# anuunchin/learned-quantization

Measured on AMD Instinct MI355X. Metric: images/sec training with fake-quant layer, CIFAR-10 bs=256, 1/2/4/8 MI355X, higher is better.
Workload: dtype f32; 1 GPU; fake-quant fwd+bwd (split) on conv-activation batch 256x3x224x224 fp32 per GPU, per_channel scales, lambda=1e-11; per_gpu_batch=256, global_batch=256, parallelism=dp1, buffer_sets=4, launch=eager

## Files before the change

learned_quantization_amd/csrc/lq_common.hpp:

```cpp
#ifndef LQ_COMMON_HPP_
#define LQ_COMMON_HPP_
#include <hip/hip_runtime.h>
#include <stdint.h>

#include "lq_hip.h"
#include "lq_fastdiv.hpp"

namespace lq {

constexpr int kBlock = 256;
constexpr int kWavesPerBlock = kBlock / 64;
constexpr float kEpsF32 = 1.1920928955078125e-07f;
constexpr int64_t kPeriodic4Min = 4ll << 20;
constexpr int64_t kNtBytes = 64ll << 20;

struct Params {
    const float* P;
    const float* s;
    const float* dy;
    float* out;
    void* q;
    int q_dtype;
    float lam;
    int tmode;
    const float* mb;
    const uint32_t* ties;
    const float* c_dev;
    float c_scale;
    int accum;
    uint32_t* pa;
    uint32_t* pb;
    double* pc;
    int64_t outer, G, inner;
    int direct;
    float* e0;
    float* e1;
    double ecount;
    float* out_perm;
    const float* dy_perm;
    float* dp_out;
    uint32_t perm_hw, perm_ci, perm_co;
};

__device__ __forceinline__ uint32_t perm_index(const Params& p, int64_t i) {
    const uint32_t iu = (uint32_t)i;
    const uint32_t t = iu / p.perm_co, o = iu - t * p.perm_co;
    const uint32_t h = t / p.perm_ci, c = t - h * p.perm_ci;
    return (o * p.perm_ci + c) * p.perm_hw + h;
}

struct FlatIdx {
    FastDiv inner, G;
};

struct Ctx {
    float s;
    float r;
    int fast;
    float k0;
    float k1;
    float lam_hi;
    int sure_ok;
};

template <typename TB, typename TC>
struct AccT {
    uint32_t a;
    TB b;
    TC c;
};
using Acc = AccT<uint32_t, double>;
using AccW = AccT<double, double>;

enum OpKind {
    OP_FWD = 0,
    OP_BWD = 1,
    OP_FUSED = 2,
    OP_MAXBIN_FWD = 3,
    OP_MAXBIN_BWD = 4,
    OP_DIFF_FWD = 5,
    OP_DIFF_BWD = 6,
    OP_QONLY = 7,
    OP_FWD_PERM = 8,
    OP_BWD_PERM = 9,
    OP_DIFF_BWD_V = 10,
};

}

#endif
```

learned_quantization_amd/csrc/lq_kernels.hip:

```cpp
#include <hip/hip_runtime.h>
#include <hip/hip_ext.h>
#include <stdarg.h>
#include <stdlib.h>
#include <stdint.h>
#include <stdio.h>
#include <string.h>

#include <new>
#include <algorithm>
#include <vector>

#include "lq_hip.h"

#include "lq_batch.hpp"
#include "lq_stream2.hpp"
#include "lq_pack.hpp"

namespace lq {

enum Mode { MODE_ROW_BIG = 0, MODE_ROW_SMALL = 1, MODE_COL = 2 };

constexpr int64_t kColRbFused = 48;
constexpr int64_t kColRbBwd = 128;

struct Plan {
    int mode;
    int64_t R, L;
    int bs;
    int CH;
    int64_t nc;
    int lpr_log2;
    int64_t C, rps, ysplit;
    int per4;
    int64_t np;
    int64_t np_ws;
    int64_t gstride, n1, stride1, n2;
};

static int64_t ceil_div(int64_t a, int64_t b) { return (a + b - 1) / b; }

#ifdef LQ_DEV_KNOBS
static int knob_env(const char* name, int dflt) {
    const char* e = getenv(name);
    return e ? atoi(e) : dflt;
}
#define LQ_KNOB(var, name, dflt) static const int var = knob_env(name, dflt)
#else
#define LQ_KNOB(var, name, dflt) constexpr int var = (dflt)
#endif

static bool flat_cols_ok(int64_t C) { return C == 8 || C == 16 || C == 32 || C == 64; }
static int64_t colx_max_inner() {
    LQ_KNOB(v, "LQ_TUNE_COLX_INNER", 200);
    return v;
}
static int64_t periodic_target() {
    LQ_KNOB(v, "LQ_TUNE_PER_NB", 2048);
    return v > 0 ? v : 2048;
}
static int64_t periodic_blocks(int64_t C) { return C * ((periodic_target() + C / 2) / C); }

static int64_t row_chunks(int64_t L, int64_t CH) {
    int64_t nc = ceil_div(L, CH);
    const int64_t r = L % CH;
    if (nc > 1 && r != 0 && r * 8 <= CH) nc -= 1;
    return nc;
}

static Plan make_plan(int64_t outer, int64_t G, int64_t inner, int force_bs = 0) {
    Plan pl;
    memset(&pl, 0, sizeof(pl));
    const int64_t N = outer * G * inner;
    int64_t R, L, f_outer;
    bool col = false;
    if (G == 1) {
        R = 1;
        L = N;
        f_outer = 1;
    } else {
        R = outer * G;
        L = inner;
        f_outer = outer;
        LQ_KNOB(colx, "LQ_TUNE_COLX", 1);
        const bool short_rows_many_layers = colx && inner >= 16 && inner < colx_max_inner() && outer >= 32 && (G * inner) % 32 == 0 &&
                                            G * inner > 64 && (double)N >= (double)kPeriodic4Min && !(inner % 4 == 0 && (inner & (inner - 1)) == 0);
        if ((inner < 16 && outer > 1) || short_rows_many_layers) {
            const int64_t C = G * inner;
            int64_t RB;
            int64_t nby = 0;
            int per4 = 0;
            if (C <= 64 && (double)outer * (double)C >= (double)kPeriodic4Min) {
                per4 = 1;
                nby = periodic_blocks(C);
                const int64_t k = 64 / C;
                RB = ceil_div(ceil_div(outer, nby), 4 * k) * 4 * k;
            } else if (C <= 64) {
                const int64_t k = 64 / C;
                RB = ceil_div(ceil_div(16384, C), 4 * k) * 4 * k;
                const int64_t rb_par = ceil_div(ceil_div(outer, 1024), 4 * k) * 4 * k;
                if (rb_par < RB) RB = rb_par;
            } else {
                RB = ceil_div(outer * ceil_div(C, 256), 512);
                RB = ceil_div(RB, 16) * 16;
                if (RB > 128) RB = 128;
                if ((double)outer * (double)C >= (double)kPeriodic4Min) RB = kColRbFused;
                if (short_rows_many_layers && ceil_div(outer, kColRbFused) * C > 2 * R) RB = kColRbBwd;
            }
            if (RB > outer) RB = outer;
            if (!nby) nby = ceil_div(outer, RB);
            if (nby * C <= R || (short_rows_many_layers && nby * C <= 2 * R)) {
                col = true;
                pl.mode = MODE_COL;
                pl.C = C;
                pl.rps = RB;
                pl.ysplit = nby;
                pl.per4 = per4;
                pl.np = nby * C;
                if (per4 && flat_cols_ok(C)) {
                    const int64_t fb = ceil_div(ceil_div(outer * C, 4) + 1, (int64_t)kFlatColsBlock * 2);
                    if (fb * C > pl.np) pl.np = fb * C;
                }
                if (C > 64 && C <= 256 && (double)outer * (double)C >= (double)kPeriodic4Min && periodic_blocks(C) * C > pl.np)
                    pl.np = periodic_blocks(C) * C;
                pl.gstride = inner;
                pl.n1 = nby;
                pl.stride1 = C;
                pl.n2 = inner;
            }
        }
    }
    if (!col) {
        pl.R = R;
// ... 53 lines not shown
static int check_hip(const char* what) {
    hipError_t e = hipGetLastError();
    if (e != hipSuccess) return fail(LQ_EHIP, "%s: %s", what, hipGetErrorString(e));
    return LQ_OK;
}

static bool aligned(const void* p, size_t a) { return (reinterpret_cast<uintptr_t>(p) % a) == 0; }

static int check_desc(int64_t outer, int64_t G, int64_t inner) {
    if (outer <= 0 || G <= 0 || inner <= 0) return fail(LQ_EINVAL, "descriptor extents must be positive (outer=%lld G=%lld inner=%lld)", (long long)outer, (long long)G, (long long)inner);
    const double n = (double)outer * (double)G * (double)inner;
    if (n > 9.0e15) return fail(LQ_EINVAL, "tensor too large");
    return LQ_OK;
}

static size_t ws_bytes_for(const Plan& pl) {
    size_t np = (size_t)(pl.np_ws > pl.np ? pl.np_ws : pl.np);
    np = (np + 63) / 64 * 64;
    return np * 16 + 256;
}

static int bind_ws(Params& p, const Plan& pl, void* ws, size_t ws_bytes) {
    if (!ws) return fail(LQ_EWORKSPACE, "workspace is NULL (need %zu bytes)", ws_bytes_for(pl));
    if (!aligned(ws, 16)) return fail(LQ_EALIGN, "workspace must be 16-byte aligned");
    if (ws_bytes < ws_bytes_for(pl)) return fail(LQ_EWORKSPACE, "workspace too small: %zu < %zu bytes", ws_bytes, ws_bytes_for(pl));
    size_t np = ((size_t)(pl.np_ws > pl.np ? pl.np_ws : pl.np) + 63) / 64 * 64;
    p.pa = reinterpret_cast<uint32_t*>(ws);
    p.pb = p.pa + np;
    p.pc = reinterpret_cast<double*>(p.pb + np);
    return LQ_OK;
}

static int row_small_lpr_log2_vec(int64_t L) {
    const int64_t l4 = L / 4;
    int lg = 0;
    while ((1 << lg) < l4 && lg < 6) ++lg;
    return lg;
}
static bool row_small_vec(const Plan& pl, const void* P, const void* dy, const void* out) {
    return pl.L % 4 == 0 && pl.L >= 8 && aligned(P, 16) && (!dy || aligned(dy, 16)) && (!out || aligned(out, 16));
}

static void col_variant(const Plan& pl, const void* P, const void* dy, const void* out, int& variant, int64_t& nbx,
                        bool allow_periodic4 = true) {
    const bool al16 = aligned(P, 16) && (!dy || aligned(dy, 16)) && (!out || aligned(out, 16));
    const double bytes = (double)pl.C * (double)pl.ysplit * (double)pl.rps * 4.0;
    if (pl.C <= 64) {
        variant = (allow_periodic4 && pl.per4 && al16) ? (bytes >= (double)kNtBytes ? 7 : 6) : 0;
        nbx = 1;
    } else if (pl.C % 4 == 0 && aligned(P, 16) && (!dy || aligned(dy, 16)) && (!out || aligned(out, 16))) {
        variant = ((double)pl.C * (double)pl.ysplit * (double)pl.rps * 4.0 >= (double)kNtBytes) ? 5 : 4;
        nbx = ceil_div(pl.C, 256);
    } else {
        variant = 1;
        nbx = ceil_div(pl.C, 64);
    }
}


#ifdef LQ_DEV_KNOBS
constexpr bool kDevKnobs = true;
#else
constexpr bool kDevKnobs = false;
#endif

template <int OP>
static int launch_stream2_impl(Plan& pl, const Params& p, hipStream_t st);

template <int OP>
static int launch_stream2(Plan& pl, const Params& p, hipStream_t st) {
    if constexpr (OP == OP_FWD || OP == OP_BWD || OP == OP_FUSED) return launch_stream2_impl<OP>(pl, p, st);
    else return 0;
}

template <int OP>
static int launch_stream2_impl(Plan& pl, const Params& p, hipStream_t st) {
    using O = OpT<OP>;
    const double numel = (double)p.outer * (double)p.G * (double)p.inner;
    if (numel < (double)kPeriodic4Min) return 0;
    if (p.out_perm || p.dy_perm) return 0;
    FlatIdx fx;
    fx.inner = make_fastdiv((uint32_t)(p.inner < 4294967296ll ? p.inner : 1));
    fx.G = make_fastdiv((uint32_t)(p.G < 4294967296ll ? p.G : 1));
    (void)fx;
    if (pl.mode == MODE_ROW_BIG) {
        if constexpr (OP == OP_FWD) {
            LQ_KNOB(off_rb, "LQ_TUNE_S2", 0);
            const int64_t nn = p.outer * p.G * p.inner;
            const bool poor_fill = (double)pl.L / (double)(pl.nc * pl.CH) < 0.95;
            if (!(off_rb & 256) && (pl.L % 32 != 0 || poor_fill || !(off_rb & 32768)) && aligned(p.P, 16) && aligned(p.out, 16)) {
                const int64_t nv = nn >> 2;
                const int rem = (int)(nn & 3);
                const int64_t blocks = ceil_div(nv + (rem ? 1 : 0), 512);
                if (blocks <= 2147483647ll) {
                    const bool ntb = numel * 4.0 >= (double)kNtBytes;
                    const bool wide = nn >= 4294967296ll;
#define LQ_FLATR(NT_, GM_) hipExtLaunchKernelGGL((k_flat_fwd<OP, 512, NT_, GM_>), dim3((unsigned)blocks), dim3(512), 0, st, g_prof_start, g_prof_stop, 0, p, fx, nv, rem)
                    if (pl.L % 4 == 0) {
                        if (ntb) { if (wide) LQ_FLATR(1, 2); else LQ_FLATR(1, 0); }
                        else LQ_FLATR(0, 0);
                    } else if (!(off_rb & 512) && (double)pl.L / (double)(pl.nc * pl.CH) >= 0.8) {
                        return 0;
                    } else {
                        if (ntb) { if (wide) LQ_FLATR(1, 7); else LQ_FLATR(1, 6); }
                        else LQ_FLATR(0, 6);
                    }
#undef LQ_FLATR
                    return check_hip("flat forward launch") ? -1 : 1;
                }
            }
        } else {
            LQ_KNOB(off_rb, "LQ_TUNE_S2", 0);
            const int nwin = (int)(pl.L % 4 ? (pl.L + 6) / 4 : pl.L / 4);
            const bool al = aligned(p.P, 16) && aligned(p.dy, 16) && (!O::kStore || aligned(p.out, 16));
            LQ_KNOB(win_max, "LQ_TUNE_WIN_MAX", 384);
            const bool wide_ok = pl.L % 4 != 0 && (double)pl.L / 2048.0 < 0.95;
            if (!(off_rb & 128) && pl.bs == 256 && pl.nc == 2 && (nwin <= win_max || wide_ok) && nwin <= 512 && al && !p.direct && pl.R < 4294967296ll) {
                const int64_t blocks = ceil_div(pl.R, (int64_t)kWavesPerBlock);
                if (blocks <= 2147483647ll) {
                    const int64_t n = p.outer * p.G * p.inner;
                    const bool ntb = numel * 4.0 >= (double)kNtBytes;
                    const FastDiv fG = make_fastdiv((uint32_t)p.G);
                    const int64_t f_outer = pl.R / p.G;
                    pl.nc = 1;
                    pl.np = pl.R;
                    pl.gstride = f_outer;
                    pl.n1 = f_outer;
                    pl.stride1 = 1;
                    pl.n2 = 1;
#define LQ_WINB(NT_, V_) hipLaunchKernelGGL((k_row_win<OP, NT_, 6, V_, 1>), dim3((unsigned)blocks), dim3(kBlock), 0, st, p, fG, pl.R, (int)pl.L, n)
                    if (nwin <= 320) { if (ntb) LQ_WINB(1, 5); else LQ_WINB(0, 5); }
                    else if (nwin <= 384) { if (ntb) LQ_WINB(1, 6); else LQ_WINB(0, 6); }
                    else if (nwin <= 448) { if (ntb) LQ_WINB(1, 7); else LQ_WINB(0, 7); }
                    else { if (ntb) LQ_WINB(1, 8); else LQ_WINB(0, 8); }
#undef LQ_WINB
                    return check_hip("row-window launch") ? -1 : 1;
                }
            }
        }
        return 0;
    }
    const bool al16 = aligned(p.P, 16) && (!O::kDy || aligned(p.dy, 16)) && (!O::kStore || aligned(p.out, 16));
    if (!al16) return 0;
    LQ_KNOB(off, "LQ_TUNE_S2", 0);
    const bool nt = numel * 4.0 >= (double)kNtBytes;
    const int64_t n = p.outer * p.G * p.inner;
    if constexpr (OP == OP_FWD) {
        const bool one_group = p.inner % 4 == 0;
        const bool scale4 = p.inner == 1 && p.G % 4 == 0 && aligned(p.s, 16) && !(off & 32);
        const bool scale4u = p.inner == 1 && p.G % 4 != 0 && p.G > 64 && !(off & 8192);
        const bool cols_pow2 = pl.mode == MODE_COL && pl.per4 && flat_cols_ok(pl.C) && !(off & 64);
        const bool straddle = pl.mode == MODE_ROW_SMALL && pl.L >= 4 && pl.L % 4 != 0 && !(off & 256);
        if (straddle) {
            const int64_t nv = n >> 2;
            const int rem = (int)(n & 3);
            const int64_t blocks = ceil_div(nv + (rem ? 1 : 0), 512);
            if (blocks <= 2147483647ll) {
                const bool wide = n >= 4294967296ll;
#define LQ_FLATS(NT_, GM_) hipLaunchKernelGGL((k_flat_fwd<OP, 512, NT_, GM_>), dim3((unsigned)blocks), dim3(512), 0, st, p, fx, nv, rem)
                if (nt) { if (wide) LQ_FLATS(1, 7); else LQ_FLATS(1, 6); }
                else LQ_FLATS(0, 6);
#undef LQ_FLATS
                return check_hip("flat forward launch") ? -1 : 1;
            }
        }
        if (scale4u && !(off & 1)) {
            const int64_t nv = n >> 2;
            const int rem = (int)(n & 3);
            const int64_t blocks = ceil_div(nv + (rem ? 1 : 0), 512);
            if (blocks <= 2147483647ll) {
                const bool wide = n >= 4294967296ll;
#define LQ_FLATU(NT_, GM_) hipLaunchKernelGGL((k_flat_fwd<OP, 512, NT_, GM_>), dim3((unsigned)blocks), dim3(512), 0, st, p, fx, nv, rem)
                if (nt) { if (wide) LQ_FLATU(1, 9); else LQ_FLATU(1, 8); }
                else LQ_FLATU(0, 8);
#undef LQ_FLATU
                return check_hip("flat forward launch") ? -1 : 1;
            }
        }
        LQ_KNOB(gather_on, "LQ_TUNE_GATHER", 1);
        if (gather_on && !(off & 1) && pl.mode == MODE_COL && !one_group && !scale4 && !scale4u && !cols_pow2 && n < 4294967296ll) {
            const int64_t nv = n >> 2;
// ... 252 lines not shown
#undef LQ_WIN
                return check_hip("row-window launch") ? -1 : 1;
            }
        }
        if ((off & 8) || pl.L > 64 || pl.L < 8 || pl.L % 4 != 0) return 0;
        const int lg = row_small_lpr_log2_vec(pl.L);
        LQ_KNOB(tiny_u, "LQ_TUNE_TINY_U", 2);
        int U = (1 << lg) < tiny_u ? (1 << lg) : tiny_u;
        if (U != 2 && U != 4) U = 2;
        const int64_t rows_per_block = (int64_t)kWavesPerBlock * (64 >> lg) * U;
        const int64_t blocks = ceil_div(pl.R, rows_per_block);
        if (blocks > 2147483647ll) return 0;
        if (pl.R >= 4294967296ll) return 0;
        const int gm = (p.outer == 1) ? 0 : 1;
#define LQ_TINY3(NT_, U_, LG_) do { \
            if (gm == 0) hipLaunchKernelGGL((k_row_tiny<OP, NT_, U_, LG_, 0>), dim3((unsigned)blocks), dim3(kBlock), 0, st, p, pl.R, (int)pl.L); \
            else hipLaunchKernelGGL((k_row_tiny<OP, NT_, U_, LG_, 1>), dim3((unsigned)blocks), dim3(kBlock), 0, st, p, pl.R, (int)pl.L); } while (0)
#ifdef LQ_DEV_KNOBS
#define LQ_TINY2(NT_) do { \
            if (lg == 1) LQ_TINY3(NT_, 2, 1); \
            else if (lg == 2) { if (U == 2) LQ_TINY3(NT_, 2, 2); else LQ_TINY3(NT_, 4, 2); } \
            else if (lg == 3) { if (U == 2) LQ_TINY3(NT_, 2, 3); else LQ_TINY3(NT_, 4, 3); } \
            else { if (U == 2) LQ_TINY3(NT_, 2, 4); else LQ_TINY3(NT_, 4, 4); } } while (0)
#else
#define LQ_TINY2(NT_) do { \
            if (lg == 1) LQ_TINY3(NT_, 2, 1); \
            else if (lg == 2) LQ_TINY3(NT_, 2, 2); \
            else if (lg == 3) LQ_TINY3(NT_, 2, 3); \
            else LQ_TINY3(NT_, 2, 4); } while (0)
#endif
        if (nt) LQ_TINY2(1); else LQ_TINY2(0);
#undef LQ_TINY2
#undef LQ_TINY3
        return check_hip("tiny-row launch") ? -1 : 1;
    }
}

template <int OP>
constexpr bool kStreamOp = OP == OP_FWD || OP == OP_BWD || OP == OP_FUSED;

template <int OP>
static int launch_traverse(Plan& pl, const Params& p, hipStream_t st) {
    using O = OpT<OP>;
    if (!kStreamOp<OP> && pl.mode == MODE_ROW_BIG && pl.bs != kBlock) return fail(LQ_EINVAL, "internal: operation %d planned with %d-thread units", OP, pl.bs);
    {
        const int r2 = launch_stream2<OP>(pl, p, st);
        if (r2 < 0) return LQ_EHIP;
        if (r2 > 0) return LQ_OK;
    }
    if (pl.mode == MODE_ROW_BIG) {
        const bool vec = aligned(p.P, 16) && (!O::kDy || aligned(p.dy, 16)) && (!O::kStore || aligned(p.out, 16));
        LQ_KNOB(tune_chunk, "LQ_TUNE_CHUNK", 1);
        LQ_KNOB(forced_bs, "LQ_TUNE_BS", 0);
        if (pl.bs == 512 && vec && tune_chunk && !p.direct && !forced_bs && pl.np_ws >= pl.R * row_chunks(pl.L, 1024)) {
            auto fill = [&](int64_t CH) { return (double)pl.L / (double)(row_chunks(pl.L, CH) * CH); };
            const bool k2_form = (OP == OP_BWD || (OP == OP_FUSED && p.tmode >= 1)) && (double)pl.R * (double)pl.L * 4.0 >= (double)kNtBytes;
            const bool small = k2_form ? (row_chunks(pl.L, 4096) > 1 && fill(1024) > fill(4096) + 0.1) : (fill(1024) > fill(2048) + 0.05);
            if (small) {
                pl.bs = 256;
                pl.CH = 1024;
                pl.nc = row_chunks(pl.L, 1024);
                pl.np = pl.R * pl.nc;
                pl.gstride = pl.nc;
                pl.stride1 = p.G * pl.nc;
                pl.n2 = pl.nc;
            }
        }
        const int64_t units = pl.R * pl.nc;
        if (units > 2147483647ll) return fail(LQ_EINVAL, "too many work units (%lld)", (long long)units);
        const int64_t outer_f = pl.R / p.G;
        const int grid3d = (p.G <= 65535 && outer_f <= 65535 && pl.R == outer_f * p.G) ? 1 : 0;
        const dim3 grid = grid3d ? dim3((unsigned)pl.nc, (unsigned)p.G, (unsigned)outer_f) : dim3((unsigned)units);
        const bool nt = kStreamOp<OP> && vec && (double)pl.R * (double)pl.L * 4.0 >= (double)kNtBytes;
        LQ_KNOB(tune_u2, "LQ_TUNE_U2", -1);
        const bool want_u2 = tune_u2 >= 0 ? tune_u2 == 1 : (OP == OP_BWD || p.tmode >= 1);
        const bool u2 = (OP == OP_BWD || OP == OP_FUSED) && want_u2 && vec && nt && pl.bs == 512;
        auto needs_tail = [&](int64_t CH) {
            const int64_t r = pl.L % CH;
            return pl.L % 4 != 0 || (pl.L > CH && r != 0 && r * 8 <= CH);
        };
        if constexpr (OP == OP_BWD || OP == OP_FUSED) if (u2) {
            const int64_t nc2 = row_chunks(pl.L, (int64_t)pl.bs * 8);
            const dim3 grid2 = grid3d ? dim3((unsigned)nc2, (unsigned)p.G, (unsigned)outer_f) : dim3((unsigned)(pl.R * nc2));
            if (needs_tail((int64_t)pl.bs * 8))
                hipExtLaunchKernelGGL((k_row_stream<OP, 4, 512, 1, 2, 1>), grid2, dim3(512), 0, st, g_prof_start, g_prof_stop, 0, p, pl.L, nc2, grid3d);
            else
                hipExtLaunchKernelGGL((k_row_stream<OP, 4, 512, 1, 2, 0>), grid2, dim3(512), 0, st, g_prof_start, g_prof_stop, 0, p, pl.L, nc2, grid3d);
            pl.CH = pl.bs * 8;
            pl.nc = nc2;
            pl.np = pl.R * nc2;
            pl.gstride = nc2;
            pl.stride1 = p.G * nc2;
            pl.n2 = nc2;
            return check_hip("traversal launch");
        }
        const bool tail1 = needs_tail((int64_t)pl.CH);
#define LQ_LAUNCH_STREAM(VEC_, BS_, NT_) do { \
        constexpr bool kTail0 = kDevKnobs || (VEC_ == 4 && !(OP == OP_FWD && (BS_ != kBlock || NT_ != 0)) && !(OP == OP_BWD && BS_ == 512 && NT_ == 1)); \
        constexpr bool kTail1 = kDevKnobs || !(OP == OP_BWD && VEC_ == 4 && BS_ == 512 && NT_ == 1); \
        if (VEC_ == 1 || tail1) { if constexpr (kTail1) hipExtLaunchKernelGGL((k_row_stream<OP, VEC_, BS_, NT_, 1, 1>), grid, dim3(BS_), 0, st, g_prof_start, g_prof_stop, 0, p, pl.L, pl.nc, grid3d); } \
        else { if constexpr (kTail0) hipExtLaunchKernelGGL((k_row_stream<OP, VEC_, BS_, NT_, 1, 0>), grid, dim3(BS_), 0, st, g_prof_start, g_prof_stop, 0, p, pl.L, pl.nc, grid3d); } } while (0)
        if constexpr (!kStreamOp<OP>) {
            if (vec) LQ_LAUNCH_STREAM(4, 256, 0);
            else LQ_LAUNCH_STREAM(1, 256, 0);
        } else if (!kDevKnobs && OP == OP_FWD && vec && !tail1 && (pl.bs != kBlock || nt)) {
            return fail(LQ_EINVAL, "internal: streaming-size forward of aligned rows reached the row stream");
        } else if (!kDevKnobs && OP == OP_BWD && vec && nt && pl.bs == 512) {
            return fail(LQ_EINVAL, "internal: streaming-size scale gradient reached the one-float4 row stream");
        } else if (vec) {
#ifdef LQ_DEV_KNOBS
            if (pl.bs == 1024) {
                if (nt) LQ_LAUNCH_STREAM(4, 1024, 1);
                else LQ_LAUNCH_STREAM(4, 1024, 0);
            } else
#endif
            if (pl.bs == 512) {
                if (nt) LQ_LAUNCH_STREAM(4, 512, 1);
                else LQ_LAUNCH_STREAM(4, 512, 0);
            } else {
                if (nt) LQ_LAUNCH_STREAM(4, 256, 1);
                else LQ_LAUNCH_STREAM(4, 256, 0);
            }
        } else {
#ifdef LQ_DEV_KNOBS
            if (pl.bs == 1024) LQ_LAUNCH_STREAM(1, 1024, 0);
            else
#endif
            if (pl.bs == 512) LQ_LAUNCH_STREAM(1, 512, 0);
            else LQ_LAUNCH_STREAM(1, 256, 0);
        }
#undef LQ_LAUNCH_STREAM
    } else if (pl.mode == MODE_ROW_SMALL) {
        const bool vec = row_small_vec(pl, p.P, O::kDy ? p.dy : nullptr, O::kStore ? p.out : nullptr);
        const int lg = vec ? row_small_lpr_log2_vec(pl.L) : pl.lpr_log2;
        const int64_t blocks = ceil_div(pl.R, kBlock >> lg);
        if (blocks > 2147483647ll) return fail(LQ_EINVAL, "too many blocks (%lld)", (long long)blocks);
        if (vec) hipLaunchKernelGGL((k_row_small<OP, 4>), dim3((unsigned)blocks), dim3(kBlock), 0, st, p, pl.R, (int)pl.L, lg);
        else hipLaunchKernelGGL((k_row_small<OP, 1>), dim3((unsigned)blocks), dim3(kBlock), 0, st, p, pl.R, (int)pl.L, lg);
    } else {
        int variant;
        int64_t nbx;
        col_variant(pl, p.P, O::kDy ? p.dy : nullptr, O::kStore ? p.out : nullptr, variant, nbx);
        const int64_t blocks = nbx * pl.ysplit;
        if (blocks > 2147483647ll) return fail(LQ_EINVAL, "too many blocks (%lld)", (long long)blocks);
        hipLaunchKernelGGL((k_col<OP>), dim3((unsigned)blocks), dim3(kBlock), 0, st, p, pl.C, pl.rps, nbx, variant, pl.ysplit);
    }
    return check_hip("traversal launch");
}

static bool finalize_cols_single(const FinGeom& f) {
    return finalize_cols_ok(f.groups, f.gstride, f.n1, f.stride1, f.n2) && f.n1 <= 64 && f.n1 * f.groups * f.n2 >= 131072;
}

template <int OP, bool COLS = true>
static int launch_finalize(const Params& p, FinGeom f, hipStream_t st) {
    const int form = finalize_form(f.groups, f.n1, f.stride1, f.n2);
    if (COLS && finalize_cols_single(f)) {
        if constexpr (COLS) hipLaunchKernelGGL((k_finalize_cols<OP>), dim3((unsigned)ceil_div(f.groups, 64 / f.n2)), dim3(kBlock), 0, st, p, f);
    } else if (form == 0) {
        hipLaunchKernelGGL((k_finalize_thread<OP>), dim3((unsigned)ceil_div(f.groups, kBlock)), dim3(kBlock), 0, st, p, f);
    } else if (form == 1) {
        hipLaunchKernelGGL((k_finalize_block<OP, 64>), dim3((unsigned)f.groups), dim3(64), 0, st, p, f);
    } else if (form == 2) {
        hipLaunchKernelGGL((k_finalize_block<OP, 256>), dim3((unsigned)f.groups), dim3(256), 0, st, p, f);
    } else {
        hipLaunchKernelGGL((k_finalize_block<OP, 1024>), dim3((unsigned)f.groups), dim3(1024), 0, st, p, f);
    }
    return check_hip("finalize launch");
}

static FinGeom group_geom(const Plan& pl, int64_t outer, int64_t G, int64_t inner) {
    FinGeom f;
    memset(&f, 0, sizeof(f));
    f.groups = G;
    f.gstride = pl.gstride;
    f.n1 = pl.n1;
    f.stride1 = pl.stride1;
    f.n2 = pl.n2;
    f.count = (double)outer * (double)inner;
    return f;
}

static FinGeom global_geom(const Plan& pl, int64_t outer, int64_t G, int64_t inner) {
    FinGeom f;
    memset(&f, 0, sizeof(f));
    f.groups = 1;
    f.gstride = 0;
    f.n1 = 1;
    f.stride1 = 0;
    f.n2 = pl.np;
    f.count = (double)outer * (double)G * (double)inner;
    return f;
}

static Params base_params(const float* P, const float* s, int64_t outer, int64_t G, int64_t inner) {
    Params p;
    memset(&p, 0, sizeof(p));
    p.P = P;
    p.s = s;
    p.outer = outer;
    p.G = G;
    p.inner = inner;
    return p;
}

static bool make_conv_tile(ConvTile& ct, int64_t hw, int64_t ci, int64_t co, int64_t outer, int64_t G, int64_t inner);
static int64_t conv_tile_partials(const ConvTile& ct, int64_t G);
static void conv_tile_fin(const ConvTile& ct, int64_t G, int64_t& gstride, int64_t& n1, int64_t& stride1, int64_t& n2);

}

using namespace lq;

#define LQ_REQUIRE_PTR(x)                                                      \
    do {                                                                       \
        if (!(x)) return fail(LQ_EINVAL, "%s: argument '%s' is NULL", __func__, #x); \
        if (!aligned((x), 4)) return fail(LQ_EALIGN, "%s: argument '%s' is not 4-byte aligned", __func__, #x); \
    } while (0)

extern "C" {

int lq_version(void) { return LQ_ABI_VERSION; }

#ifdef LQ_DEV_KNOBS
int lq_dev_set_ablate(int mask) {
    return hipMemcpyToSymbol(HIP_SYMBOL(lq::g_ablate), &mask, sizeof(int)) == hipSuccess ? LQ_OK : LQ_EHIP;
}
#endif

#ifdef LQ_DEV_KNOBS
int lq_dev_set_flags(int bits) {
    return hipMemcpyToSymbol(HIP_SYMBOL(lq::g_dev_flags), &bits, sizeof(int)) == hipSuccess ? LQ_OK : LQ_EHIP;
}
#endif

#ifdef LQ_DEV_KNOBS
int lq_dev_set_trace(void* buf) {
    unsigned long long* b = (unsigned long long*)buf;
    return hipMemcpyToSymbol(HIP_SYMBOL(lq::g_trace), &b, sizeof(b)) == hipSuccess ? LQ_OK : LQ_EHIP;
}
#endif

int lq_profile_events(void* start, void* stop) {
    g_prof_start = (hipEvent_t)start;
    g_prof_stop = (hipEvent_t)stop;
    return LQ_OK;
}

const char* lq_last_error(void) { return g_err; }

const char* lq_status_string(int status) {
    switch (status) {
        case LQ_OK: return "LQ_OK";
        case LQ_EINVAL: return "LQ_EINVAL";
        case LQ_EHIP: return "LQ_EHIP";
        case LQ_EWORKSPACE: return "LQ_EWORKSPACE";
        case LQ_EALIGN: return "LQ_EALIGN";
        default: return "LQ_UNKNOWN";
    }
}

size_t lq_workspace_bytes(int64_t outer, int64_t G, int64_t inner) {
    if (outer <= 0 || G <= 0 || inner <= 0) return 0;
    return ws_bytes_for(make_plan(outer, G, inner));
}

int lq_fq_forward(const float* P, const float* s, float* out, void* q, int q_dtype, int64_t outer, int64_t G,
                  int64_t inner, void* stream) {
    int rc = check_desc(outer, G, inner);
    if (rc) return rc;
    LQ_REQUIRE_PTR(P);
    LQ_REQUIRE_PTR(s);
    if (!out && !q) return fail(LQ_EINVAL, "lq_fq_forward: both out and q are NULL");
    if (q_dtype < LQ_Q_NONE || q_dtype > LQ_Q_I8) return fail(LQ_EINVAL, "lq_fq_forward: bad q_dtype %d", q_dtype);
    if ((q != nullptr) != (q_dtype != LQ_Q_NONE)) return fail(LQ_EINVAL, "lq_fq_forward: q and q_dtype disagree");
    Plan pl = make_plan(outer, G, inner);
    Params p = base_params(P, s, outer, G, inner);
    p.q = q;
    p.q_dtype = q_dtype;
    if (out) {
        if (!aligned(out, 4)) return fail(LQ_EALIGN, "lq_fq_forward: out is not 4-byte aligned");
        p.out = out;
        return launch_traverse<OP_FWD>(pl, p, (hipStream_t)stream);
    }
    pl = make_plan(outer, G, inner, kBlock);
    return launch_traverse<OP_QONLY>(pl, p, (hipStream_t)stream);
}

static int check_conv(const char* fn, int64_t hw, int64_t ci, int64_t co, int64_t outer, int64_t G, int64_t inner) {
    if (hw <= 0 || ci <= 0 || co <= 0) return fail(LQ_EINVAL, "%s: hw, ci, co must be positive", fn);
    const double n = (double)hw * (double)ci * (double)co;
    if (n != (double)outer * (double)G * (double)inner) return fail(LQ_EINVAL, "%s: hw*ci*co does not match the tensor", fn);
    if (n >= 4294967296.0) return fail(LQ_EINVAL, "%s: conv kernels must have fewer than 2^32 elements", fn);
    return LQ_OK;
}

int lq_fq_forward_oihw(const float* P, const float* s, float* out, float* out_oihw, int64_t hw, int64_t ci, int64_t co,
                       int64_t outer, int64_t G, int64_t inner, void* stream) {
    int rc = check_desc(outer, G, inner);
    if (rc) return rc;
    if ((rc = check_conv("lq_fq_forward_oihw", hw, ci, co, outer, G, inner))) return rc;
    LQ_REQUIRE_PTR(P);
    LQ_REQUIRE_PTR(s);
    LQ_REQUIRE_PTR(out_oihw);
    if (!out && !(aligned(P, 16) && lq_conv_tile_supported(hw, ci, co, outer, G, inner)))
        return fail(LQ_EINVAL, "lq_fq_forward_oihw: out may be NULL only for kernels the LDS-tile path takes (lq_conv_tile_supported) with P 16-byte aligned");
    Plan pl = make_plan(outer, G, inner, kBlock);
    Params p = base_params(P, s, outer, G, inner);
    p.out = out;
    p.out_perm = out_oihw;
    p.perm_hw = (uint32_t)hw;
    p.perm_ci = (uint32_t)ci;
    p.perm_co = (uint32_t)co;
    ConvTile ct;
// ... 1195 lines not shown
```

learned_quantization_amd/csrc/lq_stream2.hpp:

```cpp
#ifndef LQ_STREAM2_HPP_
#define LQ_STREAM2_HPP_
#include "lq_traverse.hpp"

namespace lq {

#ifdef LQ_DEV_KNOBS
__device__ int g_dev_flags = 0;
#endif

template <bool WIDE>
__device__ __forceinline__ int64_t flat_group_w(const Params& p, const FlatIdx& fx, int64_t i) {
    if (WIDE) return (i / p.inner) % p.G;
    return (int64_t)fd_mod(fx.G, fd_div(fx.inner, (uint32_t)i));
}
template <int GM>
__device__ __forceinline__ int64_t flat_group(const Params& p, const FlatIdx& fx, int64_t i) {
    return flat_group_w<(GM == 2 || GM == 3 || GM == 5 || GM == 7)>(p, fx, i);
}

template <int OP, int BS, int NT, int GM>
__global__ __launch_bounds__(BS) void k_flat_fwd(Params p, FlatIdx fx, int64_t nv, int rem) {
    using O = OpT<OP>;
    const int64_t v = (int64_t)blockIdx.x * BS + threadIdx.x;
    if (v < nv) {
        const int64_t i = v * 4;
        const float4 x = load4<NT>(p.P + i);
        __builtin_amdgcn_sched_barrier(0);
        Acc none = O::template init<Acc>();
        float4 o;
        if (GM == 4 || GM == 5) {
            const int64_t c = GM == 4 ? (int64_t)fd_mod(fx.G, (uint32_t)i) : i % p.G;
            const float4 sv = *reinterpret_cast<const float4*>(p.s + c);
            float4 q;
            q.x = floorf(x.x / sv.x); q.y = floorf(x.y / sv.y); q.z = floorf(x.z / sv.z); q.w = floorf(x.w / sv.w);
            o.x = q.x * sv.x; o.y = q.y * sv.y; o.z = q.z * sv.z; o.w = q.w * sv.w;
            if (p.q) {
                store_q(p.q, p.q_dtype, i + 0, q.x);
                store_q(p.q, p.q_dtype, i + 1, q.y);
                store_q(p.q, p.q_dtype, i + 2, q.z);
                store_q(p.q, p.q_dtype, i + 3, q.w);
            }
        } else if (GM == 8 || GM == 9) {
            const int64_t c = GM == 8 ? (int64_t)fd_mod(fx.G, (uint32_t)i) : i % p.G;
            float4 sv;
            if (__builtin_expect(c + 4 <= p.G, 1)) {
                sv = load4x<0, 1>(p.s + c);
            } else {
                sv.x = p.s[c];
                sv.y = p.s[c + 1 < p.G ? c + 1 : c + 1 - p.G];
                sv.z = p.s[c + 2 < p.G ? c + 2 : c + 2 - p.G];
                sv.w = p.s[c + 3 < p.G ? c + 3 : c + 3 - p.G];
            }
            float4 q;
            q.x = floorf(x.x / sv.x); q.y = floorf(x.y / sv.y); q.z = floorf(x.z / sv.z); q.w = floorf(x.w / sv.w);
            o.x = q.x * sv.x; o.y = q.y * sv.y; o.z = q.z * sv.z; o.w = q.w * sv.w;
            if (p.q) {
                store_q(p.q, p.q_dtype, i + 0, q.x);
                store_q(p.q, p.q_dtype, i + 1, q.y);
                store_q(p.q, p.q_dtype, i + 2, q.z);
                store_q(p.q, p.q_dtype, i + 3, q.w);
            }
        } else if (GM == 10 || GM == 11) {
            const uint32_t iu = (uint32_t)i;
            float4 sv;
            if (GM == 10) {
                sv.x = p.s[fd_mod(fx.G, iu)];
                sv.y = p.s[fd_mod(fx.G, iu + 1)];
                sv.z = p.s[fd_mod(fx.G, iu + 2)];
                sv.w = p.s[fd_mod(fx.G, iu + 3)];
            } else {
                sv.x = p.s[fd_mod(fx.G, fd_div(fx.inner, iu))];
                sv.y = p.s[fd_mod(fx.G, fd_div(fx.inner, iu + 1))];
                sv.z = p.s[fd_mod(fx.G, fd_div(fx.inner, iu + 2))];
                sv.w = p.s[fd_mod(fx.G, fd_div(fx.inner, iu + 3))];
            }
            float4 q;
            q.x = floorf(x.x / sv.x); q.y = floorf(x.y / sv.y); q.z = floorf(x.z / sv.z); q.w = floorf(x.w / sv.w);
            o.x = q.x * sv.x; o.y = q.y * sv.y; o.z = q.z * sv.z; o.w = q.w * sv.w;
            if (p.q) {
                store_q(p.q, p.q_dtype, i + 0, q.x);
                store_q(p.q, p.q_dtype, i + 1, q.y);
                store_q(p.q, p.q_dtype, i + 2, q.z);
                store_q(p.q, p.q_dtype, i + 3, q.w);
            }
        } else if (GM == 0 || GM == 2) {
            const Ctx ctx = O::ctx(p, flat_group<GM>(p, fx, i));
            o = O::elem4(p, ctx, i, x, x, none);
        } else if (GM == 6 || GM == 7) {
            int64_t g0, g3;
            uint32_t off6 = 0;
            int64_t off7 = 0;
            if (GM == 6) {
                const uint32_t r0 = fd_div(fx.inner, (uint32_t)i);
                off6 = (uint32_t)i - r0 * fx.inner.d;
                const uint32_t a = fd_mod(fx.G, r0), b = a + 1 == fx.G.d ? 0u : a + 1;
                g0 = a;
                g3 = off6 + 3 >= fx.inner.d ? b : a;
            } else {
                const int64_t r0 = i / p.inner;
                off7 = i - r0 * p.inner;
                g0 = r0 % p.G;
                g3 = off7 + 3 >= p.inner ? (g0 + 1 == p.G ? 0 : g0 + 1) : g0;
            }
            const float s0 = p.s[g0];
            float s3 = s0;
            if (g3 != g0) s3 = p.s[g3];
            float4 sv;
            sv.x = s0;
            sv.y = (GM == 6 ? off6 + 1 >= fx.inner.d : off7 + 1 >= p.inner) ? s3 : s0;
            sv.z = (GM == 6 ? off6 + 2 >= fx.inner.d : off7 + 2 >= p.inner) ? s3 : s0;
            sv.w = s3;
            float4 q;
            q.x = floorf(x.x / sv.x); q.y = floorf(x.y / sv.y); q.z = floorf(x.z / sv.z); q.w = floorf(x.w / sv.w);
            o.x = q.x * sv.x; o.y = q.y * sv.y; o.z = q.z * sv.z; o.w = q.w * sv.w;
            if (p.q) {
                store_q(p.q, p.q_dtype, i + 0, q.x);
                store_q(p.q, p.q_dtype, i + 1, q.y);
                store_q(p.q, p.q_dtype, i + 2, q.z);
                store_q(p.q, p.q_dtype, i + 3, q.w);
            }
        } else {
            Ctx ctx[4];
            Acc acc[4];
#pragma unroll
            for (int k = 0; k < 4; ++k) {
                ctx[k] = O::ctx(p, flat_group<GM>(p, fx, i + k));
                acc[k] = none;
            }
            o = O::elem4c(p, ctx, i, x, x, acc);
        }
        if (O::kStore) store4<NT>(p.out + i, o);
    } else if (v == nv && rem) {
        Acc none = O::template init<Acc>();
        for (int k = 0; k < rem; ++k) {
            const int64_t i = nv * 4 + k;
            const Ctx ctx = O::ctx(p, (i / p.inner) % p.G);
            const float r = O::elem(p, ctx, i, p.P[i], 0.f, none);
            if (O::kStore) p.out[i] = r;
        }
    }
}

template <int OP, int NT, int U, int NW, int UA = 0>
__global__ __launch_bounds__(NW * 64) void k_col_pipe(Params p, int64_t C, int64_t RB, int64_t nbx) {
    using O = OpT<OP>;
    __shared__ Acc lds[O::kReduce ? NW * 256 : 1];
    const int lane = threadIdx.x & 63;
    const int w = __builtin_amdgcn_readfirstlane((int)(threadIdx.x >> 6));
    int64_t b = blockIdx.x;
    if (UA >= 1 && OP == OP_BWD) {
        const int64_t nb = gridDim.x, q = nb >> 3, r = nb & 7;
        const int64_t xcd = b & 7, slot = b >> 3;
        b = (xcd < r ? xcd * (q + 1) : r * (q + 1) + (xcd - r) * q) + slot;
    }
    const int64_t by = b / nbx, bx = b - by * nbx;
    const int64_t col0n = (bx * 64 + lane) * 4;
    const bool active = col0n < C;
    const int64_t col0 = (UA == 1 && col0n + 4 > C) ? C - 4 : col0n;
    const int kdup = (int)(col0n - col0);
    const int64_t r0 = by * RB;
    const int64_t r1 = (r0 + RB < p.outer) ? r0 + RB : p.outer;
    Acc acc[4];
#pragma unroll
    for (int k = 0; k < 4; ++k) acc[k] = O::template init<Acc>();
    if (active && r0 + w < r1) {
        const int64_t step = (int64_t)NW * C;
        int64_t i0 = (r0 + w) * C + col0;
        const int cnt = (int)((r1 - (r0 + w) + NW - 1) / NW);
        const int groups = cnt / U;
        float4 xa[U], da[U], xb[U], db[U];
        if (groups > 0) {
#pragma unroll
            for (int u = 0; u < U; ++u) {
                xa[u] = load4x<NT, (UA == 1)>(p.P + i0 + u * step);
                da[u] = xa[u];
                if (O::kDy) da[u] = load4x<NT, (UA == 1)>(p.dy + i0 + u * step);
            }
        }
        __builtin_amdgcn_sched_barrier(0);
        Ctx ctx[4];
#pragma unroll
        for (int k = 0; k < 4; ++k) ctx[k] = O::ctx(p, (col0 + k) / p.inner);
        int g = 0;
        auto phase = [&](float4 (&xc)[U], float4 (&dc)[U], float4 (&xn)[U], float4 (&dn)[U]) -> bool {
            const bool more = g + 1 < groups;
            if (more) {
                const int64_t in0 = i0 + U * step;
#pragma unroll
                for (int u = 0; u < U; ++u) {
                    xn[u] = load4x<NT, (UA == 1)>(p.P + in0 + u * step);
                    dn[u] = xn[u];
                    if (O::kDy) dn[u] = load4x<NT, (UA == 1)>(p.dy + in0 + u * step);
                }
            }
            __builtin_amdgcn_sched_barrier(0);
#pragma unroll
            for (int u = 0; u < U; ++u) {
                const int64_t i = i0 + u * step;
                const float4 ov = O::elem4c(p, ctx, i, xc[u], dc[u], acc);
                if (O::kStore) store4x<NT, (UA == 1)>(p.out + i, ov);
            }
            ++g;
            i0 += U * step;
            return more;
        };
        if (groups > 0) {
            for (;;) {
                if (!phase(xa, da, xb, db)) break;
                if (!phase(xb, db, xa, da)) break;
            }
        }
        for (int t = groups * U; t < cnt; ++t) {
            const float4 x = load4x<NT, (UA == 1)>(p.P + i0);
            float4 d = x;
// ... 567 lines not shown
```

learned_quantization_amd/csrc/lq_traverse.hpp:

```cpp
#ifndef LQ_TRAVERSE_HPP_
#define LQ_TRAVERSE_HPP_
#include "lq_reduce.hpp"

namespace lq {

typedef float v4f __attribute__((ext_vector_type(4)));

template <int NT>
__device__ __forceinline__ float4 load4(const float* p) {
    if (NT) {
        const v4f v = __builtin_nontemporal_load(reinterpret_cast<const v4f*>(p));
        return make_float4(v.x, v.y, v.z, v.w);
    }
    return *reinterpret_cast<const float4*>(p);
}
template <int NT>
__device__ __forceinline__ void store4(float* p, const float4& v) {
    if (NT) {
        const v4f t = {v.x, v.y, v.z, v.w};
        __builtin_nontemporal_store(t, reinterpret_cast<v4f*>(p));
    } else {
        *reinterpret_cast<float4*>(p) = v;
    }
}

typedef float v4f_u __attribute__((ext_vector_type(4), aligned(4)));
template <int NT, int UA>
__device__ __forceinline__ float4 load4x(const float* p) {
    if (!UA) return load4<NT>(p);
    const v4f_u v = NT ? __builtin_nontemporal_load(reinterpret_cast<const v4f_u*>(p)) : *reinterpret_cast<const v4f_u*>(p);
    return make_float4(v.x, v.y, v.z, v.w);
}
template <int NT, int UA>
__device__ __forceinline__ void store4x(float* p, const float4& v) {
    if (!UA) {
        store4<NT>(p, v);
        return;
    }
    const v4f_u t = {v.x, v.y, v.z, v.w};
    if (NT) __builtin_nontemporal_store(t, reinterpret_cast<v4f_u*>(p));
    else *reinterpret_cast<v4f_u*>(p) = t;
}

template <int OP, int VEC, int BS, int NT, int U = 1, int TAIL = 1>
__device__ __forceinline__ void row_stream_body(const Params& p, int64_t L, int64_t nc, int64_t row, int64_t ck, int64_t g) {
    using O = OpT<OP>;
    constexpr int CH = BS * 4 * U;
    const int64_t base = row * L + ck * (int64_t)CH;
    const int64_t rem = L - ck * (int64_t)CH;
    const int len = (ck == nc - 1) ? (int)rem : CH;
    Acc acc = O::template init<Acc>();

    if (VEC == 4) {
        const int phase = (int)(base & 3);
        int head = (4 - phase) & 3;
        if (head > len) head = len;
        const int64_t vbase = base + head;
        const int vlen = len - head;
        const int len4 = vlen >> 2;
        int64_t i[U];
        float4 x[U], d[U];
#pragma unroll
        for (int u = 0; u < U; ++u) {
            const int j = u * BS + (int)threadIdx.x;
            i[u] = vbase + (int64_t)(j < len4 ? j : 0) * 4;
            const int64_t il = len4 > 0 ? i[u] : vbase - 4;
            x[u] = load4<NT>(p.P + il);
            d[u] = x[u];
            if (O::kDy) d[u] = load4<NT>(p.dy + il);
        }
        const bool fold = TAIL && len4 > BS * U;
        const int je = BS * U + (int)threadIdx.x;
        float4 xe = make_float4(0.f, 0.f, 0.f, 0.f), de = xe;
        if (__builtin_expect(fold && je < len4, 0)) {
            const int64_t ie0 = vbase + (int64_t)je * 4;
            xe = load4<NT>(p.P + ie0);
            de = xe;
            if (O::kDy) de = load4<NT>(p.dy + ie0);
        }
        const int tail = vlen & 3;
        const int t = (int)threadIdx.x;
        const bool edge = TAIL && (t < head || (t >= 8 && t - 8 < tail));
        const int64_t is = t < head ? base + t : vbase + (int64_t)len4 * 4 + (t - 8);
        float xs = 0.f, dsc = 0.f;
        if (edge) {
            xs = p.P[is];
            if (O::kDy) dsc = p.dy[is];
        }
        __builtin_amdgcn_sched_barrier(0);
        const Ctx ctx = O::ctx(p, g);
#pragma unroll
        for (int u = 0; u < U; ++u) {
            const int j = u * BS + (int)threadIdx.x;
            if (j < len4) {
                float4 r;
                if constexpr (O::kVec4) {
                    r = O::elem4(p, ctx, i[u], x[u], d[u], acc);
                } else {
                    r.x = O::elem(p, ctx, i[u] + 0, x[u].x, O::kDy ? d[u].x : 0.f, acc);
                    r.y = O::elem(p, ctx, i[u] + 1, x[u].y, O::kDy ? d[u].y : 0.f, acc);
                    r.z = O::elem(p, ctx, i[u] + 2, x[u].z, O::kDy ? d[u].z : 0.f, acc);
                    r.w = O::elem(p, ctx, i[u] + 3, x[u].w, O::kDy ? d[u].w : 0.f, acc);
                }
                if (O::kStore) store4<NT>(p.out + i[u], r);
            }
        }
        if (__builtin_expect(fold, 0)) {
            if (je < len4) {
                const int64_t ie = vbase + (int64_t)je * 4;
                float4 r;
                if constexpr (O::kVec4) {
                    r = O::elem4(p, ctx, ie, xe, de, acc);
                } else {
                    r.x = O::elem(p, ctx, ie + 0, xe.x, O::kDy ? de.x : 0.f, acc);
                    r.y = O::elem(p, ctx, ie + 1, xe.y, O::kDy ? de.y : 0.f, acc);
                    r.z = O::elem(p, ctx, ie + 2, xe.z, O::kDy ? de.z : 0.f, acc);
                    r.w = O::elem(p, ctx, ie + 3, xe.w, O::kDy ? de.w : 0.f, acc);
                }
                if (O::kStore) store4<NT>(p.out + ie, r);
            }
        }
        if (edge) {
            float r = O::elem(p, ctx, is, xs, dsc, acc);
            if (O::kStore) p.out[is] = r;
        }
    } else {
        float x[4 * U], d[4 * U];
#pragma unroll
        for (int u = 0; u < 4 * U; ++u) {
            const int j = u * BS + (int)threadIdx.x;
            const int jc = j < len ? j : len - 1;
            x[u] = p.P[base + jc];
            d[u] = O::kDy ? p.dy[base + jc] : 0.f;
        }
        const Ctx ctx = O::ctx(p, g);
#pragma unroll
        for (int u = 0; u < 4 * U; ++u) {
            const int j = u * BS + (int)threadIdx.x;
            if (j < len) {
                float r = O::elem(p, ctx, base + j, x[u], d[u], acc);
                if (O::kStore) p.out[base + j] = r;
            }
        }
        for (int j = 4 * U * BS + (int)threadIdx.x; j < len; j += BS) {
            float r = O::elem(p, ctx, base + j, p.P[base + j], O::kDy ? p.dy[base + j] : 0.f, acc);
            if (O::kStore) p.out[base + j] = r;
        }
    }
    if (O::kReduce) {
        [[maybe_unused]] Acc acc2;
        if constexpr (O::kSecond) acc2 = O::take_second(acc);
        if constexpr (O::kStdMerge) {
            block_reduce_dpp<BS>(acc);
        } else {
            block_reduce<O, Acc, BS>(acc);
        }
        if (threadIdx.x == 0) write_partial_t<OP>(p, row * nc + ck, acc);
        if constexpr (O::kSecond) {
            __syncthreads();
            block_reduce_dpp<BS>(acc2);
            if (threadIdx.x == 0) write_partial_second(p, row * nc + ck, acc2);
        }
    }
}

template <int OP, int VEC, int BS, int NT, int U = 1, int TAIL = 1>
__global__ __launch_bounds__(BS, (BS == 1024 ? 8 : 0)) void k_row_stream(Params p, int64_t L, int64_t nc, int grid3d) {
    int64_t row, ck, g;
    if (grid3d) {
        ck = blockIdx.x;
        g = blockIdx.y;
        row = (int64_t)blockIdx.z * p.G + g;
    } else {
        const int64_t unit = blockIdx.x;
        row = unit / nc;
        ck = unit - row * nc;
        g = row % p.G;
    }
    row_stream_body<OP, VEC, BS, NT, U, TAIL>(p, L, nc, row, ck, g);
}

template <int OP, int VEC>
__device__ __forceinline__ void row_small_body(const Params& p, int64_t R, int L, int lpr_log2, int64_t blk) {
    using O = OpT<OP>;
    const int lpr = 1 << lpr_log2;
    const int team = (int)threadIdx.x >> lpr_log2;
    const int lane = (int)threadIdx.x & (lpr - 1);
    const int64_t row = blk * (kBlock >> lpr_log2) + team;
    const bool valid = row < R;
    Acc acc = O::template init<Acc>();
    if (valid) {
        const Ctx ctx = O::ctx(p, row % p.G);
        const int64_t base = row * (int64_t)L;
        if (VEC == 4) {
            const int L4 = L >> 2;
#pragma unroll 2
            for (int j = lane; j < L4; j += lpr) {
                const int64_t i = base + (int64_t)j * 4;
                const float4 x = *reinterpret_cast<const float4*>(p.P + i);
                float4 d = x;
                if (O::kDy) d = *reinterpret_cast<const float4*>(p.dy + i);
                float4 r;
                if constexpr (O::kVec4) {
                    r = O::elem4(p, ctx, i, x, d, acc);
                } else {
                    r.x = O::elem(p, ctx, i + 0, x.x, O::kDy ? d.x : 0.f, acc);
                    r.y = O::elem(p, ctx, i + 1, x.y, O::kDy ? d.y : 0.f, acc);
                    r.z = O::elem(p, ctx, i + 2, x.z, O::kDy ? d.z : 0.f, acc);
                    r.w = O::elem(p, ctx, i + 3, x.w, O::kDy ? d.w : 0.f, acc);
                }
                if (O::kStore) *reinterpret_cast<float4*>(p.out + i) = r;
            }
        } else {
#pragma unroll 4
            for (int j = lane; j < L; j += lpr) {
                const float x = p.P[base + j];
                const float d = O::kDy ? p.dy[base + j] : 0.f;
                float r = O::elem(p, ctx, base + j, x, d, acc);
                if (O::kStore) p.out[base + j] = r;
            }
        }
    }
    if (O::kReduce) {
        [[maybe_unused]] Acc acc2;
        if constexpr (O::kSecond) {
            acc2 = O::take_second(acc);
            wave_reduce<O>(acc2, lpr);
        }
        wave_reduce<O>(acc, lpr);
        if (valid && lane == 0) {
            const int64_t o = row / p.G, g = row - o * p.G;
            write_partial_t<OP>(p, (p.G > 1 ? g * p.outer + o : row), acc);
            if constexpr (O::kSecond) write_partial_second(p, (p.G > 1 ? g * p.outer + o : row), acc2);
        }
    }
}

template <int OP, int VEC>
__global__ __launch_bounds__(kBlock) void k_row_small(Params p, int64_t R, int L, int lpr_log2) {
    row_small_body<OP, VEC>(p, R, L, lpr_log2, (int64_t)blockIdx.x);
}

constexpr int kColUnroll = 4;

template <class O>
__device__ __forceinline__ void col_cross_wave(Acc* lds, const Acc& mine, int slot, int slots) {
    lds[(threadIdx.x >> 6) * slots + slot] = mine;
}

template <int OP, int VW, int NT>
__device__ __forceinline__ void col_tile_body(const Params& p, int64_t C, int64_t RB, int64_t bx, int64_t by, Acc* lds) {
    using O = OpT<OP>;
    const int lane = threadIdx.x & 63, w = threadIdx.x >> 6;
    const int64_t col0 = (bx * 64 + lane) * VW;
    const bool active = col0 < C;
    Ctx ctx[VW];
    Acc acc[VW];
#pragma unroll
    for (int k = 0; k < VW; ++k) {
        acc[k] = O::template init<Acc>();
        ctx[k] = O::ctx(p, active ? (col0 + k) / p.inner : 0);
    }
// ... 477 lines not shown
```

Before: 2.601 million images/s.

## Keep forward tail of P in MALL and walk backward in reverse

For large streaming tensors, the forward flat kernel now loads the last ~44 MB of P with the default cache policy and writes its output with sc1 nt stores, so that data can stay resident in the last-level MALL/Infinity Cache. The split backward row-stream kernel (U=2 path) then walks blocks in reverse order and uses default-policy loads for that same tail region. The goal is for backward to hit cache on the portion of P that forward touched last, cutting HBM reads. The risk is added cache pollution and an index remap, and the benefit depends on how large the MALL is and on what runs between the two kernels.

```diff
diff --git a/learned_quantization_amd/csrc/lq_common.hpp b/learned_quantization_amd/csrc/lq_common.hpp
--- a/learned_quantization_amd/csrc/lq_common.hpp
+++ b/learned_quantization_amd/csrc/lq_common.hpp
@@ -13,6 +13,7 @@
 constexpr float kEpsF32 = 1.1920928955078125e-07f;
 constexpr int64_t kPeriodic4Min = 4ll << 20;
 constexpr int64_t kNtBytes = 64ll << 20;
+constexpr int64_t kMallKeepBytes = 44ll << 20;
 
 struct Params {
     const float* P;
@@ -51,6 +52,7 @@
 
 struct FlatIdx {
     FastDiv inner, G;
+    uint32_t keep_from;
 };
 
 struct Ctx {
diff --git a/learned_quantization_amd/csrc/lq_kernels.hip b/learned_quantization_amd/csrc/lq_kernels.hip
--- a/learned_quantization_amd/csrc/lq_kernels.hip
+++ b/learned_quantization_amd/csrc/lq_kernels.hip
@@ -48,6 +48,20 @@
 #else
 #define LQ_KNOB(var, name, dflt) constexpr int var = (dflt)
 #endif
+
+#ifdef LQ_DEV_KNOBS
+static int g_dev_flags_host = 0;
+#endif
+static int64_t mall_keep_from(int64_t numel) {
+    int64_t keep = kMallKeepBytes / 4;
+    LQ_KNOB(t_env, "LQ_TUNE_MALL_T", 0);
+    int t = t_env;
+#ifdef LQ_DEV_KNOBS
+    if (g_dev_flags_host & 0xf00) t = (g_dev_flags_host >> 8) & 15;
+#endif
+    if (t > 0) keep = (int64_t)((double)numel * (t - 1) / 10.0);
+    return keep >= numel ? 0 : numel - keep;
+}
 
 static bool flat_cols_ok(int64_t C) { return C == 8 || C == 16 || C == 32 || C == 64; }
 static int64_t colx_max_inner() {
@@ -267,6 +281,7 @@
     FlatIdx fx;
     fx.inner = make_fastdiv((uint32_t)(p.inner < 4294967296ll ? p.inner : 1));
     fx.G = make_fastdiv((uint32_t)(p.G < 4294967296ll ? p.G : 1));
+    fx.keep_from = 0xffffffffu;
     (void)fx;
     if (pl.mode == MODE_ROW_BIG) {
         if constexpr (OP == OP_FWD) {
@@ -282,6 +297,7 @@
                     const bool wide = nn >= 4294967296ll;
 #define LQ_FLATR(NT_, GM_) hipExtLaunchKernelGGL((k_flat_fwd<OP, 512, NT_, GM_>), dim3((unsigned)blocks), dim3(512), 0, st, g_prof_start, g_prof_stop, 0, p, fx, nv, rem)
                     if (pl.L % 4 == 0) {
+                        if (ntb) fx.keep_from = (uint32_t)ceil_div(mall_keep_from(nn), 2048);
                         if (ntb) { if (wide) LQ_FLATR(1, 2); else LQ_FLATR(1, 0); }
                         else LQ_FLATR(0, 0);
                     } else if (!(off_rb & 512) && (double)pl.L / (double)(pl.nc * pl.CH) >= 0.8) {
@@ -700,10 +716,14 @@
         if constexpr (OP == OP_BWD || OP == OP_FUSED) if (u2) {
             const int64_t nc2 = row_chunks(pl.L, (int64_t)pl.bs * 8);
             const dim3 grid2 = grid3d ? dim3((unsigned)nc2, (unsigned)p.G, (unsigned)outer_f) : dim3((unsigned)(pl.R * nc2));
+            int64_t keep_from = OP == OP_BWD ? mall_keep_from(pl.R * pl.L) : 0;
+#ifdef LQ_DEV_KNOBS
+            if (g_dev_flags_host & 0x1000) keep_from = -1 - keep_from;
+#endif
             if (needs_tail((int64_t)pl.bs * 8))
-                hipExtLaunchKernelGGL((k_row_stream<OP, 4, 512, 1, 2, 1>), grid2, dim3(512), 0, st, g_prof_start, g_prof_stop, 0, p, pl.L, nc2, grid3d);
+                hipExtLaunchKernelGGL((k_row_stream<OP, 4, 512, 1, 2, 1>), grid2, dim3(512), 0, st, g_prof_start, g_prof_stop, 0, p, pl.L, nc2, grid3d, keep_from);
             else
-                hipExtLaunchKernelGGL((k_row_stream<OP, 4, 512, 1, 2, 0>), grid2, dim3(512), 0, st, g_prof_start, g_prof_stop, 0, p, pl.L, nc2, grid3d);
+                hipExtLaunchKernelGGL((k_row_stream<OP, 4, 512, 1, 2, 0>), grid2, dim3(512), 0, st, g_prof_start, g_prof_stop, 0, p, pl.L, nc2, grid3d, keep_from);
             pl.CH = pl.bs * 8;
             pl.nc = nc2;
             pl.np = pl.R * nc2;
@@ -716,8 +736,8 @@
 #define LQ_LAUNCH_STREAM(VEC_, BS_, NT_) do { \
         constexpr bool kTail0 = kDevKnobs || (VEC_ == 4 && !(OP == OP_FWD && (BS_ != kBlock || NT_ != 0)) && !(OP == OP_BWD && BS_ == 512 && NT_ == 1)); \
         constexpr bool kTail1 = kDevKnobs || !(OP == OP_BWD && VEC_ == 4 && BS_ == 512 && NT_ == 1); \
-        if (VEC_ == 1 || tail1) { if constexpr (kTail1) hipExtLaunchKernelGGL((k_row_stream<OP, VEC_, BS_, NT_, 1, 1>), grid, dim3(BS_), 0, st, g_prof_start, g_prof_stop, 0, p, pl.L, pl.nc, grid3d); } \
-        else { if constexpr (kTail0) hipExtLaunchKernelGGL((k_row_stream<OP, VEC_, BS_, NT_, 1, 0>), grid, dim3(BS_), 0, st, g_prof_start, g_prof_stop, 0, p, pl.L, pl.nc, grid3d); } } while (0)
+        if (VEC_ == 1 || tail1) { if constexpr (kTail1) hipExtLaunchKernelGGL((k_row_stream<OP, VEC_, BS_, NT_, 1, 1>), grid, dim3(BS_), 0, st, g_prof_start, g_prof_stop, 0, p, pl.L, pl.nc, grid3d, (int64_t)0); } \
+        else { if constexpr (kTail0) hipExtLaunchKernelGGL((k_row_stream<OP, VEC_, BS_, NT_, 1, 0>), grid, dim3(BS_), 0, st, g_prof_start, g_prof_stop, 0, p, pl.L, pl.nc, grid3d, (int64_t)0); } } while (0)
         if constexpr (!kStreamOp<OP>) {
             if (vec) LQ_LAUNCH_STREAM(4, 256, 0);
             else LQ_LAUNCH_STREAM(1, 256, 0);
@@ -848,6 +868,7 @@
 
 #ifdef LQ_DEV_KNOBS
 int lq_dev_set_flags(int bits) {
+    g_dev_flags_host = bits;
     return hipMemcpyToSymbol(HIP_SYMBOL(lq::g_dev_flags), &bits, sizeof(int)) == hipSuccess ? LQ_OK : LQ_EHIP;
 }
 #endif
diff --git a/learned_quantization_amd/csrc/lq_stream2.hpp b/learned_quantization_amd/csrc/lq_stream2.hpp
--- a/learned_quantization_amd/csrc/lq_stream2.hpp
+++ b/learned_quantization_amd/csrc/lq_stream2.hpp
@@ -22,9 +22,12 @@
 __global__ __launch_bounds__(BS) void k_flat_fwd(Params p, FlatIdx fx, int64_t nv, int rem) {
     using O = OpT<OP>;
     const int64_t v = (int64_t)blockIdx.x * BS + threadIdx.x;
+    constexpr bool kKeep = NT == 1 && (GM == 0 || GM == 2);
     if (v < nv) {
         const int64_t i = v * 4;
-        const float4 x = load4<NT>(p.P + i);
+        float4 x;
+        if (kKeep && blockIdx.x >= fx.keep_from) x = load4_keep(p.P + i);
+        else x = load4<NT>(p.P + i);
         __builtin_amdgcn_sched_barrier(0);
         Acc none = O::template init<Acc>();
         float4 o;
@@ -129,7 +132,12 @@
             }
             o = O::elem4c(p, ctx, i, x, x, acc);
         }
-        if (O::kStore) store4<NT>(p.out + i, o);
+#ifdef LQ_DEV_KNOBS
+        if (O::kStore && kKeep && (g_dev_flags & 0x70)) store4_policy((g_dev_flags >> 4) & 7, p.out + i, o);
+        else
+#endif
+        if (O::kStore && kKeep) store4_sc1nt(p.out + i, o);
+        else if (O::kStore) store4<NT>(p.out + i, o);
     } else if (v == nv && rem) {
         Acc none = O::template init<Acc>();
         for (int k = 0; k < rem; ++k) {
diff --git a/learned_quantization_amd/csrc/lq_traverse.hpp b/learned_quantization_amd/csrc/lq_traverse.hpp
--- a/learned_quantization_amd/csrc/lq_traverse.hpp
+++ b/learned_quantization_amd/csrc/lq_traverse.hpp
@@ -24,7 +24,30 @@
     }
 }
 
+__device__ __forceinline__ void store4_sc1nt(float* p, const float4& v) {
+    const v4f t = {v.x, v.y, v.z, v.w};
+    asm volatile("global_store_dwordx4 %0, %1, off sc1 nt" : : "v"(p), "v"(t) : "memory");
+}
+#ifdef LQ_DEV_KNOBS
+__device__ __forceinline__ void store4_policy(int pol, float* p, const float4& v) {
+    const v4f t = {v.x, v.y, v.z, v.w};
+    if (pol == 1) asm volatile("global_store_dwordx4 %0, %1, off" : : "v"(p), "v"(t) : "memory");
+    else if (pol == 2) asm volatile("global_store_dwordx4 %0, %1, off sc1 nt" : : "v"(p), "v"(t) : "memory");
+    else if (pol == 3) asm volatile("global_store_dwordx4 %0, %1, off sc0 sc1 nt" : : "v"(p), "v"(t) : "memory");
+    else if (pol == 4) asm volatile("global_store_dwordx4 %0, %1, off sc1" : : "v"(p), "v"(t) : "memory");
+    else if (pol == 5) asm volatile("global_store_dwordx4 %0, %1, off sc0 sc1" : : "v"(p), "v"(t) : "memory");
+    else __builtin_nontemporal_store(t, reinterpret_cast<v4f*>(p));
+}
+#endif
+
 typedef float v4f_u __attribute__((ext_vector_type(4), aligned(4)));
+__device__ __forceinline__ float4 load4_keep(const float* p) {
+    asm volatile("; default-policy load" : : : );
+    const v4f_u v = *reinterpret_cast<const v4f_u*>(p);
+    asm volatile("; end" : : : );
+    return make_float4(v.x, v.y, v.z, v.w);
+}
+
 template <int NT, int UA>
 __device__ __forceinline__ float4 load4x(const float* p) {
     if (!UA) return load4<NT>(p);
@@ -42,11 +65,16 @@
     else *reinterpret_cast<v4f_u*>(p) = t;
 }
 
+template <int OP, int VEC, int NT, int U>
+constexpr bool kMallWalk = OP == OP_BWD && VEC == 4 && NT == 1 && U == 2;
+
 template <int OP, int VEC, int BS, int NT, int U = 1, int TAIL = 1>
-__device__ __forceinline__ void row_stream_body(const Params& p, int64_t L, int64_t nc, int64_t row, int64_t ck, int64_t g) {
+__device__ __forceinline__ void row_stream_body(const Params& p, int64_t L, int64_t nc, int64_t row, int64_t ck, int64_t g,
+                                                int64_t keep_from = 0) {
     using O = OpT<OP>;
     constexpr int CH = BS * 4 * U;
     const int64_t base = row * L + ck * (int64_t)CH;
+    [[maybe_unused]] const bool keep = kMallWalk<OP, VEC, NT, U> && base >= keep_from;
     const int64_t rem = L - ck * (int64_t)CH;
     const int len = (ck == nc - 1) ? (int)rem : CH;
     Acc acc = O::template init<Acc>();
@@ -65,7 +93,8 @@
             const int j = u * BS + (int)threadIdx.x;
             i[u] = vbase + (int64_t)(j < len4 ? j : 0) * 4;
             const int64_t il = len4 > 0 ? i[u] : vbase - 4;
-            x[u] = load4<NT>(p.P + il);
+            if (kMallWalk<OP, VEC, NT, U> && keep) x[u] = load4_keep(p.P + il);
+            else x[u] = load4<NT>(p.P + il);
             d[u] = x[u];
             if (O::kDy) d[u] = load4<NT>(p.dy + il);
         }
@@ -165,19 +194,26 @@
 }
 
 template <int OP, int VEC, int BS, int NT, int U = 1, int TAIL = 1>
-__global__ __launch_bounds__(BS, (BS == 1024 ? 8 : 0)) void k_row_stream(Params p, int64_t L, int64_t nc, int grid3d) {
+__global__ __launch_bounds__(BS, (BS == 1024 ? 8 : 0)) void k_row_stream(Params p, int64_t L, int64_t nc, int grid3d, int64_t keep_from) {
+    constexpr bool kRev = kMallWalk<OP, VEC, NT, U>;
+#ifdef LQ_DEV_KNOBS
+    const bool rev = kRev && keep_from >= 0;
+    if (kRev && !rev) keep_from = -1 - keep_from;
+#else
+    constexpr bool rev = kRev;
+#endif
     int64_t row, ck, g;
     if (grid3d) {
-        ck = blockIdx.x;
-        g = blockIdx.y;
-        row = (int64_t)blockIdx.z * p.G + g;
+        ck = rev ? gridDim.x - 1 - blockIdx.x : blockIdx.x;
+        g = rev ? gridDim.y - 1 - blockIdx.y : blockIdx.y;
+        row = (int64_t)(rev ? gridDim.z - 1 - blockIdx.z : blockIdx.z) * p.G + g;
     } else {
-        const int64_t unit = blockIdx.x;
+        const int64_t unit = rev ? gridDim.x - 1 - blockIdx.x : blockIdx.x;
         row = unit / nc;
         ck = unit - row * nc;
         g = row % p.G;
     }
-    row_stream_body<OP, VEC, BS, NT, U, TAIL>(p, L, nc, row, ck, g);
+    row_stream_body<OP, VEC, BS, NT, U, TAIL>(p, L, nc, row, ck, g, keep_from);
 }
 
 template <int OP, int VEC>
```

Measured after the change: 2.677 million images/s (median of 6 runs). 1.03x the previous value.
